# OPTML-Group/Unlearn-Saliency

Measured on AMD Instinct MI355X. Metric: unlearn_steps_per_sec (ResNet-18/CIFAR-10 10%-forget, RL + SalUn mask, batch 256/GPU), higher is better.
Workload: dtype f32

## Files before the change

### include/salun.h

```cpp
#ifndef SALUN_H
#define SALUN_H

#include <stddef.h>
#include <stdint.h>

#ifdef __cplusplus
extern "C" {
#endif

#define SALUN_OK 0
#define SALUN_EINVAL (-22)
#define SALUN_ENOSPC (-28)
#define SALUN_EIO (-5)

#define SALUN_MAX_THRESHOLDS 16

typedef void *salun_stream_t;

int salun_version(void);
const char *salun_strerror(int code);
const char *salun_arch(void);
int salun_clock_probe(unsigned long long *out , int samples, int spins, salun_stream_t stream);

int salun_saliency_accumulate(float *acc , const float *g ,
// ... 163 lines not shown
                       float *lse , int B, int H, int Nq, int Nk, int D, long long q_bs, int q_ld,
                       long long k_bs, int k_ld, long long v_bs, int v_ld, long long o_bs, int o_ld, double scale,
                       salun_stream_t stream);
int salun_attn_backward(const uint16_t *q , const uint16_t *k , const uint16_t *v ,
                        const uint16_t *o , const uint16_t *d_o , const float *lse ,
                        uint16_t *dq , uint16_t *dk , uint16_t *dv , float *dsum , int B, int H,
                        int Nq, int Nk, int D, long long q_bs, int q_ld, long long k_bs, int k_ld, long long v_bs, int v_ld,
                        long long o_bs, int o_ld, long long do_bs, int do_ld, double scale, salun_stream_t stream);

size_t salun_ln_bf16_workspace_bytes(int64_t rows, int C);
int salun_ln_bf16_forward(const uint16_t *x , const float *gamma , const float *beta ,
                          uint16_t *y , float *stats , int64_t rows, int C, double eps,
                          salun_stream_t stream);
int salun_ln_bf16_backward(const uint16_t *dy , const uint16_t *x , const float *gamma ,
                           const float *stats , uint16_t *dx , float *dgamma , float *dbeta ,
                           int64_t rows, int C, int accumulate, void *ws , size_t ws_bytes, salun_stream_t stream);
int salun_geglu_bf16_forward(const uint16_t *h , uint16_t *out , int64_t rows, int F, salun_stream_t stream);
int salun_geglu_bf16_backward(const uint16_t *h , const uint16_t *dy , uint16_t *dh , int64_t rows,
                              int F, salun_stream_t stream);

size_t salun_bn_workspace_bytes(int C);
int salun_bn_forward(const float *x , const float *res , float *y ,
                     const float *gamma , const float *beta , float *running_mean ,
                     float *running_var , long long *num_batches_tracked ,
                     float *save_mean , float *save_invstd ,
                     int N, int C, int HW, int training, double momentum, double eps, int relu, void *ws ,
                     size_t ws_bytes, salun_stream_t stream);
int salun_bn_backward(const float *dy , const float *y , const float *x ,
                      const float *gamma , const float *save_mean , const float *save_invstd ,
                      float *dx , float *dres , float *dgamma , float *dbeta ,
                      float *grad_gamma_acc , float *grad_beta_acc ,
                      int N, int C, int HW, int training, int relu, void *ws , size_t ws_bytes,
                      salun_stream_t stream);

size_t salun_gn_workspace_bytes(int N, int C);
int salun_gn_forward(const float *x , float *y , const float *gamma , const float *beta ,
                     float *save_mean , float *save_rstd , int N, int C, int HW, int G, double eps,
                     int silu, salun_stream_t stream);
int salun_gn_backward(const float *dz , const float *x , const float *gamma ,
                      const float *beta , const float *save_mean , const float *save_rstd ,
                      float *dx , float *dgamma , float *dbeta ,
                      float *grad_gamma_acc , float *grad_beta_acc ,
                      int N, int C, int HW, int G, int silu, void *ws , size_t ws_bytes,
                      salun_stream_t stream);

int salun_gn_backward_fused(const float *dz , const float *x , const float *gamma ,
                            const float *beta , const float *save_mean , const float *save_rstd ,
                            const float *addend , float *dx , float *dgamma ,
                            float *dbeta , float *grad_gamma_acc ,
                            float *grad_beta_acc , float *nk_sum ,
                            float *csum , float *csum_acc , int N, int C, int HW, int G,
                            int silu, void *ws , size_t ws_bytes, salun_stream_t stream);

int salun_param_diff(const float *p , const float *p0 , float *out , int64_t n,
                     salun_stream_t stream);
int salun_soft_threshold_step(float *p , const float *p0 , const float *tau ,
                              int64_t n, salun_stream_t stream);

size_t salun_ewc_workspace_bytes(int64_t n);
int salun_ewc_penalty_grad(const float *p , const float *p_star , const float *F ,
                           float *g , double lambda, float *loss_out , int64_t n,
                           void *ws , size_t ws_bytes, salun_stream_t stream);

int salun_image_batch(const uint8_t *data , const int64_t *idx ,
                      const int32_t *crop , const uint8_t *flip ,
                      float *out , int64_t B, int H, int W, int C, int pad,
// ... 149 lines not shown
```

### unlearn_saliency_amd/_lib.py

```python
from __future__ import annotations

import ctypes
import os
import subprocess

_HERE = os.path.dirname(os.path.abspath(__file__))
LIB_PATH = os.environ.get("SALUN_LIB") or os.path.join(_HERE, "libsalun.so")
CSRC_DIR = os.path.join(_HERE, "csrc")

SALUN_OK = 0
SALUN_EINVAL = -22
SALUN_ENOSPC = -28
SALUN_EIO = -5
SALUN_MAX_THRESHOLDS = 16
SALUN_TOPK_FORCE_FULL_SCAN = 1
SALUN_TOPK_VALUES_ONLY = 2
SALUN_WGRAD_SHARED = 1

c_void_p, c_int, c_int64, c_uint64 = ctypes.c_void_p, ctypes.c_int, ctypes.c_int64, ctypes.c_uint64
c_double, c_size_t = ctypes.c_double, ctypes.c_size_t

class GemmSeg(ctypes.Structure):
    _fields_ = [("A", c_void_p), ("B", c_void_p), ("K", ctypes.c_int32), ("a_i", ctypes.c_int32),
                ("a_k", ctypes.c_int32), ("b_j", ctypes.c_int32), ("b_k", ctypes.c_int32)]
# ... 79 lines not shown
    "salun_conv3x3_pack_weights": (c_int, [c_void_p, c_int, c_void_p]),
    "salun_conv3x3_packed": (c_int, [c_void_p] * 6 + [c_int] * 6 + [c_void_p]),
    "salun_conv2d_backward_weight": (c_int, [c_void_p, c_void_p, c_void_p] + [c_int] * 11 + [c_void_p, c_size_t,
                                                                                          c_void_p]),
    "salun_conv2d_backward_weight_ex": (c_int, [c_void_p, c_void_p, c_void_p] + [c_int] * 11 + [ctypes.c_uint, c_void_p,
                                                                                                 c_size_t, c_void_p]),
    "salun_conv2d_route": (c_int, [c_int] * 11 + [ctypes.c_uint, c_size_t, ctypes.c_char_p, c_size_t,
                                   ctypes.POINTER(c_int)]),
    "salun_conv2d_bf16_supported": (c_int, [c_int] * 5),
    "salun_conv2d_bf16_pack_weights": (c_int, [c_void_p, c_void_p, c_int, c_int, c_int, c_void_p]),
    "salun_bf16_pack_weights_batch": (c_int, [c_void_p, c_int, c_void_p]),
    "salun_conv2d_bf16_data_workspace_bytes": (c_size_t, [c_int] * 8),
    "salun_conv2d_bf16_forward": (c_int, [c_void_p] * 6 + [c_int] * 8 + [c_void_p, c_size_t, c_void_p]),
    "salun_conv2d_bf16_backward_data": (c_int, [c_void_p] * 4 + [c_int] * 8 + [c_void_p, c_size_t, c_void_p]),
    "salun_conv2d_bf16_wgrad_workspace_bytes": (c_size_t, [c_int] * 8),
    "salun_conv2d_bf16_backward_weight": (c_int, [c_void_p] * 4 + [c_int] * 9 + [c_void_p, c_size_t, c_void_p]),
    "salun_colsum_bf16_workspace_bytes": (c_size_t, [c_int]),
    "salun_colsum_bf16": (c_int, [c_void_p, c_void_p, c_void_p, c_int64, c_int, c_int, c_int, c_void_p, c_size_t, c_void_p]),
    "salun_conv2d_bf16_backward_weight_ex": (c_int, [c_void_p] * 5 + [c_int] * 9 + [c_void_p, c_size_t, c_void_p]),
    "salun_gn_bf16_workspace_bytes": (c_size_t, [c_int] * 4),
    "salun_gn_bf16_forward": (c_int, [c_void_p] * 6 + [c_int] * 4 + [c_double, c_int, c_void_p, c_size_t, c_void_p]),
    "salun_gn_bf16_backward": (c_int, [c_void_p] * 8 + [c_int] * 6 + [c_void_p, c_size_t, c_void_p]),
    "salun_attn_supported": (c_int, [c_int]),
    "salun_attn_forward": (c_int, [c_void_p] * 5 + [c_int] * 5 + [ctypes.c_longlong, c_int] * 4 + [c_double, c_void_p]),
    "salun_attn_backward": (c_int, [c_void_p] * 10 + [c_int] * 5 + [ctypes.c_longlong, c_int] * 5 + [c_double, c_void_p]),
    "salun_ln_bf16_workspace_bytes": (c_size_t, [c_int64, c_int]),
    "salun_ln_bf16_forward": (c_int, [c_void_p] * 5 + [c_int64, c_int, c_double, c_void_p]),
    "salun_ln_bf16_backward": (c_int, [c_void_p] * 7 + [c_int64, c_int, c_int, c_void_p, c_size_t, c_void_p]),
    "salun_geglu_bf16_forward": (c_int, [c_void_p, c_void_p, c_int64, c_int, c_void_p]),
    "salun_geglu_bf16_backward": (c_int, [c_void_p, c_void_p, c_void_p, c_int64, c_int, c_void_p]),
    "salun_bn_workspace_bytes": (c_size_t, [c_int]),
    "salun_bn_forward": (c_int, [c_void_p] * 10 + [c_int] * 4 + [c_double, c_double, c_int, c_void_p, c_size_t, c_void_p]),
    "salun_bn_backward": (c_int, [c_void_p] * 12 + [c_int] * 5 + [c_void_p, c_size_t, c_void_p]),
    "salun_conv2d_backward_data_add": (c_int, [c_void_p] * 4 + [c_int] * 10 + [c_void_p]),
    "salun_gn_workspace_bytes": (c_size_t, [c_int, c_int]),
    "salun_gn_forward": (c_int, [c_void_p] * 6 + [c_int] * 4 + [c_double, c_int, c_void_p]),
    "salun_gn_backward": (c_int, [c_void_p] * 11 + [c_int] * 5 + [c_void_p, c_size_t, c_void_p]),
    "salun_gn_backward_fused": (c_int, [c_void_p] * 15 + [c_int] * 5 + [c_void_p, c_size_t, c_void_p]),
    "salun_param_diff": (c_int, [c_void_p, c_void_p, c_void_p, c_int64, c_void_p]),
    "salun_soft_threshold_step": (c_int, [c_void_p, c_void_p, c_void_p, c_int64, c_void_p]),
    "salun_ewc_workspace_bytes": (c_size_t, [c_int64]),
    "salun_ewc_penalty_grad": (c_int, [c_void_p] * 4 + [c_double, c_void_p, c_int64, c_void_p, c_size_t, c_void_p]),
    "salun_image_batch": (c_int, [c_void_p, c_void_p, c_void_p, c_void_p, c_void_p, c_int64, c_int, c_int, c_int,
                                  c_int, c_void_p]),
    "salun_gemm_f32_workspace_bytes": (c_size_t, [ctypes.POINTER(GemmJob), c_int, ctypes.POINTER(GemmSeg), c_int, c_int,
                                                  c_int]),
    "salun_gemm_f32": (c_int, [ctypes.POINTER(GemmJob), c_int, ctypes.POINTER(GemmSeg), c_int, c_int, c_int,
                               ctypes.POINTER(c_int64), c_double, c_void_p, c_size_t, c_void_p]),
    "salun_gemm_f32_route": (c_int, [ctypes.POINTER(GemmJob), c_int, ctypes.POINTER(GemmSeg), c_int, c_int, c_int,
                                     ctypes.POINTER(c_int64), c_void_p, c_size_t, ctypes.POINTER(GemmRoute)]),
    "salun_colsum_f32_workspace_bytes": (c_size_t, [c_int64, c_int]),
    "salun_colsum_f32": (c_int, [c_void_p, c_void_p, c_int64, c_int, c_int64, c_int, c_void_p, c_size_t, c_void_p]),
    "salun_softmax_rows": (c_int, [c_void_p, c_int64, c_int, c_int, c_void_p]),
    "salun_softmax_rows_backward": (c_int, [c_void_p, c_void_p, c_int64, c_int, c_int, c_double, c_void_p]),
    "salun_gemm_bf16_supported": (c_int, [c_int64, c_int, c_int]),
    "salun_gemm_bf16_nt": (c_int, [c_void_p, c_void_p, c_void_p, c_void_p, c_void_p, c_int64, c_int, c_int, c_int, c_void_p]),
    "salun_pack_bf16": (c_int, [c_void_p, c_void_p, c_int, c_int, c_int, c_void_p]),
    "salun_gemm_bf16_tn_supported": (c_int, [c_int64, c_int, c_int]),
    "salun_gemm_bf16_tn_workspace_bytes": (c_size_t, [c_int64, c_int, c_int, c_int]),
    "salun_gemm_bf16_tn": (c_int, [c_void_p, c_void_p, c_void_p, c_int64, c_int, c_int, c_int, c_int, c_void_p, c_size_t, c_void_p]),
    "salun_dropout": (c_int, [c_void_p, c_void_p, c_int64, c_int64, c_int64, c_double, c_uint64, c_void_p, c_void_p]),
    "salun_u64_add": (c_int, [c_void_p, c_uint64, c_void_p]),
    "salun_iu_dot_workspace_bytes": (c_size_t, [c_int, c_int64]),
    "salun_iu_conv_dot": (c_int, [c_void_p, c_void_p, c_int, c_int64, c_void_p, c_void_p, c_size_t, c_void_p]),
    "salun_iu_bn_dot": (c_int, [c_void_p] * 4 + [c_double] + [c_void_p] * 4 + [c_int] * 3 + [c_void_p, c_void_p,
                                                                                           c_size_t, c_void_p]),
# ... 75 lines not shown
```

### unlearn_saliency_amd/csrc/salun_norm.hip

```cpp
#include "salun_common.h"

namespace {

constexpr int BN_MAX_SPLIT = 64;


struct BnWalk {
  int n, i, dn, di, hw4;
  __device__ __forceinline__ BnWalk(int n_lo, int hw4_) : hw4(hw4_) {
    const int t = threadIdx.x;
    n = n_lo + t / hw4_;
    i = t - (t / hw4_) * hw4_;
    dn = 256 / hw4_;
    di = 256 - dn * hw4_;
  }
  __device__ __forceinline__ void next() {
    n += dn;
    i += di;
    if (i >= hw4) { i -= hw4; ++n; }
  }
};

__global__ __launch_bounds__(256) void k_bn_stats_partial(const float *__restrict__ x, int N, int C, int HW, int nsplit,
                                                          double *__restrict__ partial) {
  __shared__ double lds[4];
  const int c = blockIdx.x, s = blockIdx.y;
  const int n_lo = (int)((int64_t)N * s / nsplit), n_hi = (int)((int64_t)N * (s + 1) / nsplit);
  float s1 = 0.f, s2 = 0.f;
  double d1 = 0.0, d2 = 0.0;
  const int hw4 = HW >> 2;
  const int work = (n_hi - n_lo) * hw4;
  int it = 0;
// ... 168 lines not shown
  __syncthreads();
  const float mu = mean[c], is = invstd[c];
  const float gi = gamma[c] * is;
  const float kb = sg[0] * inv_m, kg = sg[1] * inv_m;
  const int n_lo = (int)((int64_t)N * s / nsplit), n_hi = (int)((int64_t)N * (s + 1) / nsplit);
  const int hw4 = HW >> 2;
  const int work = (n_hi - n_lo) * hw4;
  BnWalk wk(n_lo, hw4);
#pragma unroll 2
  for (int e = threadIdx.x; e < work; e += 256, wk.next()) {
    const int n = wk.n, i = wk.i;
    const size_t off = ((size_t)n * C + c) * HW;
    float4 g = reinterpret_cast<const float4 *>(dy + off)[i];
    if (RELU) {
      const float4 yv = reinterpret_cast<const float4 *>(y + off)[i];
      g.x = yv.x > 0.f ? g.x : 0.f; g.y = yv.y > 0.f ? g.y : 0.f;
      g.z = yv.z > 0.f ? g.z : 0.f; g.w = yv.w > 0.f ? g.w : 0.f;
    }
    if (DRES) reinterpret_cast<float4 *>(dres + off)[i] = g;
    float4 o;
    if (TRAIN) {
      const float4 xv = reinterpret_cast<const float4 *>(x + off)[i];
      o.x = gi * (g.x - (kb + ((xv.x - mu) * is) * kg));
      o.y = gi * (g.y - (kb + ((xv.y - mu) * is) * kg));
      o.z = gi * (g.z - (kb + ((xv.z - mu) * is) * kg));
      o.w = gi * (g.w - (kb + ((xv.w - mu) * is) * kg));
    } else {
      o.x = gi * g.x; o.y = gi * g.y; o.z = gi * g.z; o.w = gi * g.w;
    }
    reinterpret_cast<float4 *>(dx + off)[i] = o;
  }
}

inline int bn_nsplit(int N, int C) {
  int ns = (1024 + C - 1) / C;
  if (ns > N) ns = N;
  if (ns > BN_MAX_SPLIT) ns = BN_MAX_SPLIT;
  if (ns < 1) ns = 1;
  return ns;
}

}

SALUN_EXPORT size_t salun_bn_workspace_bytes(int C) {
  return sizeof(double) * 2 * (size_t)(C > 0 ? C : 0) * BN_MAX_SPLIT;
}

SALUN_EXPORT int salun_bn_forward(const float *x, const float *res, float *y, const float *gamma, const float *beta,
                                  float *running_mean, float *running_var, long long *num_batches_tracked,
                                  float *save_mean, float *save_invstd, int N, int C, int HW, int training,
                                  double momentum, double eps, int relu, void *ws, size_t ws_bytes,
                                  salun_stream_t stream) {
  if (!x || !y || !gamma || !beta || !save_mean || !save_invstd || N < 1 || C < 1 || HW < 4 || (HW & 3))
    return SALUN_EINVAL;
  if (!training && (!running_mean || !running_var)) return SALUN_EINVAL;
  if (!salun_aligned16(x) || !salun_aligned16(y) || (res && !salun_aligned16(res))) return SALUN_EINVAL;
  hipStream_t st = salun_hip_stream(stream);
  const int ns = bn_nsplit(N, C);
  double *partial = static_cast<double *>(ws);
  if (training) {
    if (!ws || ws_bytes < salun_bn_workspace_bytes(C)) return SALUN_ENOSPC;
    hipLaunchKernelGGL(k_bn_stats_partial, dim3(C, ns), dim3(256), 0, st, x, N, C, HW, ns, partial);
    SALUN_LAUNCH_CHECK();
  }
#define SALUN_BN_APPLY(RELU_, RES_, TRAIN_)                                                                       \
  hipLaunchKernelGGL((k_bn_apply<RELU_, RES_, TRAIN_>), dim3(C, ns), dim3(256), 0, st, x, res, y, partial,         \
                     save_mean, save_invstd, gamma, beta, running_mean, running_var, num_batches_tracked, N, C,  \
                     HW, ns, (float)eps, (float)momentum)
  const bool r = relu != 0, a = res != nullptr, t = training != 0;
  if (r && a && t) SALUN_BN_APPLY(true, true, true);
  else if (r && a) SALUN_BN_APPLY(true, true, false);
  else if (r && t) SALUN_BN_APPLY(true, false, true);
  else if (r) SALUN_BN_APPLY(true, false, false);
  else if (a && t) SALUN_BN_APPLY(false, true, true);
  else if (a) SALUN_BN_APPLY(false, true, false);
  else if (t) SALUN_BN_APPLY(false, false, true);
  else SALUN_BN_APPLY(false, false, false);
#undef SALUN_BN_APPLY
// ... 8 lines not shown
                                   salun_stream_t stream) {
  if (!dy || !x || !gamma || !save_mean || !save_invstd || !dx || !dgamma || !dbeta || N < 1 || C < 1 || HW < 4 ||
      (HW & 3) || (relu && !y))
    return SALUN_EINVAL;
  if (!ws || ws_bytes < salun_bn_workspace_bytes(C)) return SALUN_ENOSPC;
  if (!salun_aligned16(dy) || !salun_aligned16(x) || !salun_aligned16(dx) || (y && !salun_aligned16(y)) ||
      (dres && !salun_aligned16(dres)))
    return SALUN_EINVAL;
  hipStream_t st = salun_hip_stream(stream);
  const int ns = bn_nsplit(N, C);
  double *partial = static_cast<double *>(ws);
  if (relu) hipLaunchKernelGGL(k_bn_bwd_partial<true>, dim3(C, ns), dim3(256), 0, st, dy, y, x, save_mean, save_invstd, N, C, HW, ns, partial);
  else hipLaunchKernelGGL(k_bn_bwd_partial<false>, dim3(C, ns), dim3(256), 0, st, dy, y, x, save_mean, save_invstd, N, C, HW, ns, partial);
  SALUN_LAUNCH_CHECK();
  const float inv_m = (float)(1.0 / ((double)N * HW));
#define SALUN_BN_BWD(RELU_, TRAIN_, DRES_)                                                                          \
  hipLaunchKernelGGL((k_bn_bwd_apply<RELU_, TRAIN_, DRES_>), dim3(C, ns), dim3(256), 0, st, dy, y, x, save_mean,   \
                     save_invstd, gamma, partial, dgamma, dbeta, grad_gamma_acc, grad_beta_acc, dx, dres, N, C, HW, \
                     ns, inv_m)
  const bool r = relu != 0, t = training != 0, d = dres != nullptr;
  if (r && t && d) SALUN_BN_BWD(true, true, true);
  else if (r && t) SALUN_BN_BWD(true, true, false);
  else if (r && d) SALUN_BN_BWD(true, false, true);
  else if (r) SALUN_BN_BWD(true, false, false);
  else if (t && d) SALUN_BN_BWD(false, true, true);
  else if (t) SALUN_BN_BWD(false, true, false);
  else if (d) SALUN_BN_BWD(false, false, true);
  else SALUN_BN_BWD(false, false, false);
#undef SALUN_BN_BWD
  SALUN_LAUNCH_CHECK();
  return SALUN_OK;
}

namespace {

constexpr int GN_ITEMS = 16;
constexpr int GN_MAX_SEG = 1024;

__device__ __forceinline__ float gn_sigmoid(float y) { return 1.0f / (1.0f + expf(-y)); }

__device__ __forceinline__ float seg_sum(float v, int r) {
  for (int off = 1; off < r; off <<= 1) v += __shfl_xor(v, off, 64);
  return v;
}

template <bool SILU, int ITEMS>
__global__ __launch_bounds__(256) void k_gn_fwd(const float *__restrict__ x, float *__restrict__ y,
                                                const float *__restrict__ gamma, const float *__restrict__ beta,
                                                float *__restrict__ mean, float *__restrict__ rstd, int C, int HW,
                                                int G, float eps) {
  constexpr bool CACHED = ITEMS > 0;
  __shared__ double lds[4];
  __shared__ float st[2];
  const int ng = blockIdx.x, n = ng / G, g = ng - n * G;
  const int cpg = C / G;
  const int L = cpg * HW, nvec = L >> 2;
  const size_t base = ((size_t)n * C + (size_t)g * cpg) * HW;
  const float4 *xv = reinterpret_cast<const float4 *>(x + base);
  float4 v[CACHED ? ITEMS : 1];
  float s1 = 0.f, s2 = 0.f;
  double d1 = 0.0, d2 = 0.0;
  if (CACHED) {
#pragma unroll
    for (int i = 0; i < (CACHED ? ITEMS : 1); ++i) {
      const int e = threadIdx.x + i * 256;
      if (e < nvec) v[i] = xv[e];
// ... 349 lines not shown
```

### unlearn_saliency_amd/norm.py

```python
from __future__ import annotations

import torch

from .fastfn import FastFunction
import torch.nn as nn
import torch.nn.functional as F

from . import gradsink, ops


class _FusedBN(FastFunction):
    @staticmethod
    def forward(ctx, x, weight, bias, residual, running_mean, running_var, training, momentum, eps, relu, nbt=None):
        out = ops.bn_forward(x, residual, weight, bias, running_mean, running_var, training, momentum, eps, relu, nbt)
        if out is None:
            raise RuntimeError("fused BN: unsupported shape (H*W must be a multiple of 4)")
        y, mean, invstd = out
        ctx.save_for_backward(x, y if relu else None, weight, bias, mean, invstd)
        ctx.params = (weight, bias)
        ctx.cfg = (bool(training), bool(relu), residual is not None)
        ctx.mark_non_differentiable(mean, invstd)
        return y

    @staticmethod
    def backward(ctx, dy):
        x, y, weight, bias, mean, invstd = ctx.saved_tensors
        training, relu, has_res = ctx.cfg
        gw, gb = gradsink.sink(ctx.params[0]), gradsink.sink(ctx.params[1])
        if gw is None or gb is None:
            gw = gb = None
        dx, dres, dgamma, dbeta = ops.bn_backward(_grad_on_grid(dy), y, x, weight, mean, invstd, training, relu,
                                                  has_res and ctx.needs_input_grad[3], gw, gb)
        if gw is not None:
            gradsink.arrived(weight)
            gradsink.arrived(bias)
            dgamma = dbeta = None
        return dx, dgamma, dbeta, dres, None, None, None, None, None, None, None


def _on_grid(t: torch.Tensor) -> bool:
    return t.data_ptr() % 16 == 0


def _grad_on_grid(dy: torch.Tensor) -> torch.Tensor:
    dy = dy.contiguous()
    return dy if _on_grid(dy) else dy.clone()


def _eligible(x: torch.Tensor, bn: nn.BatchNorm2d) -> bool:
    return (type(bn) is nn.BatchNorm2d and x.is_cuda and x.dtype == torch.float32 and x.dim() == 4 and (x.shape[2] * x.shape[3]) % 4 == 0
            and bn.affine and bn.track_running_stats and bn.momentum is not None and not torch.is_autocast_enabled())


def fused_bn_act(x: torch.Tensor, bn: nn.BatchNorm2d, residual: torch.Tensor = None, relu: bool = True):
    ok = _eligible(x, bn) and (not x.is_contiguous() or _on_grid(x)) and \
        (residual is None or not residual.is_contiguous() or _on_grid(residual))
    if not ok:
        y = bn(x)
        if residual is not None:
            y = y + residual
        return F.relu(y) if relu else y
    x = x.contiguous()
    if residual is not None:
        residual = residual.contiguous()
    return _FusedBN.apply(x, bn.weight, bn.bias, residual, bn.running_mean, bn.running_var, bn.training,
# ... 91 lines not shown
```

### unlearn_saliency_amd/ops.py

```python
from __future__ import annotations

import ctypes
from typing import Optional, Sequence

import torch

from .fastfn import FastFunction

from . import _lib, ringpack, weightimg
from ._lib import c_double, c_int, c_int64, c_size_t, c_uint64, c_void_p, check
from .streams import _stream, _stream_handle


def _dev(t: Optional[torch.Tensor], dtype: torch.dtype, name: str, allow_none: bool = False) -> c_void_p:
    if t is None:
        if allow_none:
            return c_void_p(None)
        raise ValueError(f"{name} must not be None")
    if not t.is_cuda:
        raise RuntimeError(f"{name}: the SalUn HIP kernels need a device tensor (got {t.device}); no CPU fallback")
    if t.dtype != dtype:
        raise TypeError(f"{name}: expected {dtype}, got {t.dtype}")
    if not t.is_contiguous():
        raise ValueError(f"{name} must be contiguous")
# ... 787 lines not shown
                            _dev(gamma, torch.float32, "weight"), _dev(beta, torch.float32, "bias"),
                            _dev(running_mean, torch.float32, "running_mean", True),
                            _dev(running_var, torch.float32, "running_var", True),
                            _dev(num_batches_tracked, torch.int64, "num_batches_tracked", True),
                            c_void_p(mean.data_ptr()),
                            c_void_p(invstd.data_ptr()), N, C, H * W, int(bool(training)), c_double(momentum),
                            c_double(eps), int(bool(relu)), c_void_p(ws.data_ptr()), c_size_t(ws.numel()), _stream())
    if rc == _lib.SALUN_EINVAL:
        return None
    check(rc, "salun_bn_forward")
    return y, mean, invstd


def bn_backward(dy, y, x, gamma, mean, invstd, training, relu, want_dres, gamma_grad_acc=None, beta_grad_acc=None):
    N, C, H, W = x.shape
    L = _lib.lib()
    dx = torch.empty_like(x)
    dres = torch.empty_like(x) if want_dres else None
    dgamma = torch.empty(C, dtype=torch.float32, device=x.device)
    dbeta = torch.empty(C, dtype=torch.float32, device=x.device)
    ws = workspace(L.salun_bn_workspace_bytes(C), x.device)
    check(L.salun_bn_backward(_dev(dy, torch.float32, "dy"), _dev(y, torch.float32, "y", True),
                              _dev(x, torch.float32, "x"), _dev(gamma, torch.float32, "weight"),
                              _dev(mean, torch.float32, "mean"), _dev(invstd, torch.float32, "invstd"),
                              c_void_p(dx.data_ptr()), _dev(dres, torch.float32, "dres", True),
                              c_void_p(dgamma.data_ptr()), c_void_p(dbeta.data_ptr()),
                              _dev(gamma_grad_acc, torch.float32, "gamma.grad", True),
                              _dev(beta_grad_acc, torch.float32, "beta.grad", True), N, C, H * W,
                              int(bool(training)), int(bool(relu)), c_void_p(ws.data_ptr()), c_size_t(ws.numel()),
                              _stream()), "salun_bn_backward")
    return dx, dres, dgamma, dbeta


def gn_forward(x, gamma, beta, groups, eps, silu):
    N, C, H, W = x.shape
    z = torch.empty_like(x)
    mean = torch.empty(N * groups, dtype=torch.float32, device=x.device)
    rstd = torch.empty(N * groups, dtype=torch.float32, device=x.device)
    rc = _lib.lib().salun_gn_forward(_dev(x, torch.float32, "x"), c_void_p(z.data_ptr()),
                                     _dev(gamma, torch.float32, "weight"), _dev(beta, torch.float32, "bias"),
                                     c_void_p(mean.data_ptr()), c_void_p(rstd.data_ptr()), N, C, H * W, int(groups),
                                     c_double(eps), int(bool(silu)), _stream())
    if rc == _lib.SALUN_EINVAL:
        return None
    check(rc, "salun_gn_forward")
    return z, mean, rstd


def gn_backward(dz, x, gamma, beta, mean, rstd, groups, silu, gamma_grad_acc=None, beta_grad_acc=None, addend=None,
                nk_sum: bool = False, csum: bool = False, csum_acc=None):
    N, C, H, W = x.shape
    L = _lib.lib()
    dx = torch.empty_like(x)
    dgamma = torch.empty(C, dtype=torch.float32, device=x.device)
    dbeta = torch.empty(C, dtype=torch.float32, device=x.device)
    ws = workspace(L.salun_gn_workspace_bytes(N, C), x.device)
    if addend is not None and addend.shape != x.shape:
        raise ValueError("gn_backward: addend must have the shape of x")
    want_nk = bool(nk_sum or csum or csum_acc is not None)
    nk = torch.empty((N, C), dtype=torch.float32, device=x.device) if want_nk else None
    cs = torch.empty(C, dtype=torch.float32, device=x.device) if csum else None
    check(L.salun_gn_backward_fused(_dev(dz, torch.float32, "dz"), _dev(x, torch.float32, "x"),
                                    _dev(gamma, torch.float32, "weight"), _dev(beta, torch.float32, "bias"),
                                    _dev(mean, torch.float32, "mean"), _dev(rstd, torch.float32, "rstd"),
                                    _dev(addend, torch.float32, "addend", True),
                                    c_void_p(dx.data_ptr()), c_void_p(dgamma.data_ptr()), c_void_p(dbeta.data_ptr()),
# ... 124 lines not shown
```

### unlearn_saliency_amd/resblock.py

```python
from __future__ import annotations

import torch

from .fastfn import FastFunction
import torch.nn as nn

import os

from . import dist as sdist
from . import draws, gradsink, ops, wgrad_side

FWD_SHORTCUT_BESIDE = os.environ.get("SALUN_FWD_SHORTCUT_BESIDE", "1") != "0"


def _bn_args(bn: nn.BatchNorm2d):
    return bn.running_mean, bn.running_var, bn.training, bn.momentum, bn.eps


class _BasicBlockFn(FastFunction):
    @staticmethod
    def forward(ctx, x, blk, w1, g1, b1, w2, g2, b2, wd, gd, bd):
        s = blk.conv1.stride[0]
        N, C, H, W = x.shape
        P, Q = (H + 2 - 3) // s + 1, (W + 2 - 3) // s + 1
        training = blk.bn1.training
        cd = md = idd = None
        fork = None
        if wd is not None:
            def shortcut():
                cd_ = ops.conv2d_forward(x, wd, None, s, 0, P, Q)
                return (cd_,) + tuple(ops.bn_forward(cd_, None, gd, bd, *_bn_args(blk.downsample[1]), False,
                                                     blk.downsample[1].num_batches_tracked))
            if (FWD_SHORTCUT_BESIDE and wgrad_side.OVERLAP and x.is_cuda
                    and not torch.cuda.is_current_stream_capturing()):
                main, fork = torch.cuda.current_stream(x.device), wgrad_side.stream(x.device)
                fork.wait_stream(main)
                with torch.cuda.stream(fork):
                    cd, skip, md, idd = shortcut()
                x.record_stream(fork)
        c1 = ops.conv2d_forward(x, w1, None, s, 1, P, Q)
        y1, m1, i1 = ops.bn_forward(c1, None, g1, b1, *_bn_args(blk.bn1), True, blk.bn1.num_batches_tracked)
        c2 = ops.conv2d_forward(y1, w2, None, 1, 1, P, Q)
        if wd is None:
            skip = x
        elif fork is None:
            cd, skip, md, idd = shortcut()
        else:
            main.wait_stream(fork)
            for t in (cd, skip, md, idd):
                if t is not None:
                    t.record_stream(main)
        out, m2, i2 = ops.bn_forward(c2, skip, g2, b2, *_bn_args(blk.bn2), True, blk.bn2.num_batches_tracked)
        ctx.save_for_backward(x, c1, y1, c2, out, cd, w1, g1, b1, w2, g2, b2, wd, gd, bd, m1, i1, m2, i2, md, idd)
        ctx.cfg = (s, training)
        return out

    @staticmethod
    def backward(ctx, dout):
        x, c1, y1, c2, out, cd, w1, g1, b1, w2, g2, b2, wd, gd, bd, m1, i1, m2, i2, md, idd = ctx.saved_tensors
        s, training = ctx.cfg
        dout = dout.contiguous()
        grads = {}

        def bn_bwd(dy, y, xin, g, b, m, i, relu, want_dres):
            gw, gb = gradsink.sink(g), gradsink.sink(b)
            if gw is None or gb is None:
                gw = gb = None
            dx, dres, dg, db = ops.bn_backward(dy, y, xin, g, m, i, training, relu, want_dres, gw, gb)
            if gw is not None:
                gradsink.arrived(g)
                gradsink.arrived(b)
                dg = db = None
            return dx, dres, dg, db

        dev = dout.device
        overlap = wgrad_side.OVERLAP

        def wgrad(xin, dy, w, stride, pad):
            dst = gradsink.sink(w)
            if overlap:
                dw = wgrad_side.beside(dev, (xin, dy), lambda side: ops.conv2d_backward_weight(
                    xin, dy, w.shape, stride, pad, out=dst, accumulate=True, shared=True, stream=side), alloc=dst is None)
            else:
                dw = ops.conv2d_backward_weight(xin, dy, w.shape, stride, pad, out=dst, accumulate=True)
            if dst is not None:
                gradsink.arrived(w)
                return None
            return dw

        dc2, dskip, dg2, db2 = bn_bwd(dout, out, c2, g2, b2, m2, i2, True, True)
        dwd = dgd = dbd = None
        dxd = dskip
        if wd is not None:
            dcd, _, dgd, dbd = bn_bwd(dskip, None, cd, gd, bd, md, idd, False, False)
            dwd = wgrad(x, dcd, wd, s, 0)
            dxd = ops.conv2d_backward_data(dcd, wd, x.shape, s, 0) if ctx.needs_input_grad[0] else None
        dw2 = wgrad(y1, dc2, w2, 1, 1)
        dy1 = ops.conv2d_backward_data(dc2, w2, y1.shape, 1, 1)
        dc1, _, dg1, db1 = bn_bwd(dy1, y1, c1, g1, b1, m1, i1, True, False)
        dw1 = wgrad(x, dc1, w1, s, 1)
        dx = ops.conv2d_backward_data(dc1, w1, x.shape, s, 1, addend=dxd) if ctx.needs_input_grad[0] else None
        if overlap and not all(g is None for g in (dw1, dw2, dwd)):
            torch.cuda.current_stream(dev).wait_stream(wgrad_side.stream(dev))
            wgrad_side.release_held(dev)
        return dx, None, dw1, dg1, db1, dw2, dg2, db2, dwd, dgd, dbd


def _probe(blk, shape, device) -> bool:
    N, C, H, W = shape
    s = blk.conv1.stride[0]
    P, Q = (H + 2 - 3) // s + 1, (W + 2 - 3) // s + 1
    K = blk.conv1.out_channels
    if (P * Q) % 4 or (H * W) % 4:
        return False
    e = lambda *sh: torch.empty(sh, dtype=torch.float32, device=device)
    x, y1, dy = e(N, C, H, W), e(N, K, P, Q), e(N, K, P, Q)
    convs = [(x, blk.conv1.weight, s, 1), (y1, blk.conv2.weight, 1, 1)]
    if blk.downsample is not None:
        convs.append((x, blk.downsample[0].weight, s, 0))
    for xin, w, st, pad in convs:
        if ops.conv2d_forward(xin, w, None, st, pad, P, Q) is None:
            return False
        if ops.conv2d_backward_data(dy, w, xin.shape, st, pad, addend=xin) is None:
            return False
        if ops.conv2d_backward_weight(xin, dy, w.shape, st, pad) is None:
            return False
    return True


def _structure_ok(blk) -> bool:
    convs = [blk.conv1, blk.conv2] + ([blk.downsample[0]] if blk.downsample is not None else [])
    bns = [blk.bn1, blk.bn2] + ([blk.downsample[1]] if blk.downsample is not None else [])
# ... 207 lines not shown
```

Before: 117.7.

## Store BN+ReLU activation masks as ballot bitmasks and read them in backward

The fused BN forward kernels now write a per-wave ballot bitmask of positive ReLU outputs, and the backward kernels read these bits instead of the saved f32 output tensor to mask the incoming gradient. This replaces a full-size activation read in the BN backward passes with a much smaller bitmask read. It adds small bitmask writes in forward and more kernel variants. In the residual block the full output tensors are still saved alongside the bits, so memory use grows slightly.

```diff
diff --git a/include/salun.h b/include/salun.h
--- a/include/salun.h
+++ b/include/salun.h
@@ -219,6 +219,20 @@
                       float *grad_gamma_acc , float *grad_beta_acc ,
                       int N, int C, int HW, int training, int relu, void *ws , size_t ws_bytes,
                       salun_stream_t stream);
+size_t salun_bn_relu_bits_bytes(int N, int C, int HW);
+int salun_bn_forward_bits(const float *x , const float *res , float *y ,
+                          const float *gamma , const float *beta , float *running_mean ,
+                          float *running_var , long long *num_batches_tracked ,
+                          float *save_mean , float *save_invstd , void *relu_bits ,
+                          size_t relu_bits_bytes, int N, int C, int HW, int training, double momentum, double eps,
+                          int relu, void *ws , size_t ws_bytes, salun_stream_t stream);
+int salun_bn_backward_bits(const float *dy , const void *relu_bits ,
+                           size_t relu_bits_bytes, const float *x , const float *gamma ,
+                           const float *save_mean , const float *save_invstd , float *dx ,
+                           float *dres , float *dgamma , float *dbeta ,
+                           float *grad_gamma_acc ,
+                           float *grad_beta_acc , int N, int C, int HW, int training,
+                           int relu, void *ws , size_t ws_bytes, salun_stream_t stream);
 
 size_t salun_gn_workspace_bytes(int N, int C);
 int salun_gn_forward(const float *x , float *y , const float *gamma , const float *beta ,
diff --git a/unlearn_saliency_amd/_lib.py b/unlearn_saliency_amd/_lib.py
--- a/unlearn_saliency_amd/_lib.py
+++ b/unlearn_saliency_amd/_lib.py
@@ -135,6 +135,11 @@
     "salun_bn_workspace_bytes": (c_size_t, [c_int]),
     "salun_bn_forward": (c_int, [c_void_p] * 10 + [c_int] * 4 + [c_double, c_double, c_int, c_void_p, c_size_t, c_void_p]),
     "salun_bn_backward": (c_int, [c_void_p] * 12 + [c_int] * 5 + [c_void_p, c_size_t, c_void_p]),
+    "salun_bn_relu_bits_bytes": (c_size_t, [c_int] * 3),
+    "salun_bn_forward_bits": (c_int, [c_void_p] * 11 + [c_size_t] + [c_int] * 4 + [c_double, c_double, c_int, c_void_p,
+                                                                                 c_size_t, c_void_p]),
+    "salun_bn_backward_bits": (c_int, [c_void_p] * 2 + [c_size_t] + [c_void_p] * 10 + [c_int] * 5 + [c_void_p, c_size_t,
+                                                                                                     c_void_p]),
     "salun_conv2d_backward_data_add": (c_int, [c_void_p] * 4 + [c_int] * 10 + [c_void_p]),
     "salun_gn_workspace_bytes": (c_size_t, [c_int, c_int]),
     "salun_gn_forward": (c_int, [c_void_p] * 6 + [c_int] * 4 + [c_double, c_int, c_void_p]),
diff --git a/unlearn_saliency_amd/csrc/salun_norm.hip b/unlearn_saliency_amd/csrc/salun_norm.hip
--- a/unlearn_saliency_amd/csrc/salun_norm.hip
+++ b/unlearn_saliency_amd/csrc/salun_norm.hip
@@ -1,3 +1,5 @@
+#include <type_traits>
+
 #include "salun_common.h"
 
 namespace {
@@ -232,6 +234,248 @@
   }
 }
 
+struct BnWaveWalk {
+  int full, all;
+  size_t word0;
+  __device__ __forceinline__ BnWaveWalk(int work, int c, int s, int nsplit, int max_it) {
+    const int lo = __builtin_amdgcn_readfirstlane((int)(threadIdx.x & ~63u));
+    all = work > lo ? (work - lo + 255) >> 8 : 0;
+    full = work > lo + 63 ? (work - lo - 63 + 255) >> 8 : 0;
+    word0 = (((size_t)c * nsplit + s) * max_it) * 16 + (size_t)(lo >> 6) * 4;
+  }
+};
+
+template <int U>
+struct BnItems : std::integral_constant<int, U> {};
+
+__device__ __forceinline__ float bn_keep(unsigned long long m, float g) {
+  float r;
+  asm("v_cndmask_b32_e64 %0, 0, %1, %2" : "=v"(r) : "v"(g), "s"(m));
+  return r;
+}
+
+__device__ __forceinline__ float4 bn_keep4(const unsigned long long *__restrict__ w, float4 g) {
+  g.x = bn_keep(w[0], g.x); g.y = bn_keep(w[1], g.y); g.z = bn_keep(w[2], g.z); g.w = bn_keep(w[3], g.w);
+  return g;
+}
+
+template <bool RES, bool TRAIN>
+__global__ __launch_bounds__(256) void k_bn_apply_bits(const float *__restrict__ x, const float *__restrict__ res,
+                                                       float *__restrict__ y, const double *__restrict__ partial,
+                                                       float *__restrict__ mean, float *__restrict__ invstd,
+                                                       const float *__restrict__ gamma,
+                                                       const float *__restrict__ beta,
+                                                       float *__restrict__ running_mean,
+                                                       float *__restrict__ running_var,
+                                                       long long *__restrict__ num_batches_tracked, int N, int C,
+                                                       int HW, int nsplit, float eps, float momentum,
+                                                       unsigned long long *__restrict__ bits, int max_it) {
+  __shared__ float st[2];
+  const int c = blockIdx.x, s = blockIdx.y;
+  if (TRAIN) {
+    if (num_batches_tracked && c == 0 && s == 0 && threadIdx.x == 0) *num_batches_tracked += 1;
+    bn_channel_stats(partial, c, nsplit, (double)N * HW, eps, st, s == 0, momentum, mean, invstd, running_mean,
+                     running_var);
+  } else {
+    if (threadIdx.x == 0) {
+      st[0] = running_mean[c];
+      st[1] = 1.0f / sqrtf(running_var[c] + eps);
+      if (s == 0) { mean[c] = st[0]; invstd[c] = st[1]; }
+    }
+    __syncthreads();
+  }
+  const float a = st[1] * gamma[c];
+  const float b = beta[c] - st[0] * a;
+  const int n_lo = (int)((int64_t)N * s / nsplit), n_hi = (int)((int64_t)N * (s + 1) / nsplit);
+  const int hw4 = HW >> 2;
+  const int work = (n_hi - n_lo) * hw4;
+  BnWalk wk(n_lo, hw4);
+  const BnWaveWalk ww(work, c, s, nsplit, max_it);
+  unsigned long long *__restrict__ words = bits + ww.word0;
+  int it = 0;
+  auto step = [&](auto items, const bool partial_it) {
+    constexpr int U = decltype(items)::value;
+    const bool in = !partial_it || (int)threadIdx.x + 256 * it < work;
+    size_t off[U];
+    int pi[U];
+    float4 v[U] = {}, r[U] = {}, o[U];
+    unsigned long long m[U][4];
+#pragma unroll
+    for (int u = 0; u < U; ++u, wk.next()) {
+      off[u] = ((size_t)wk.n * C + c) * HW;
+      pi[u] = wk.i;
+    }
+    if (in) {
+#pragma unroll
+      for (int u = 0; u < U; ++u) {
+        v[u] = reinterpret_cast<const float4 *>(x + off[u])[pi[u]];
+        if (RES) r[u] = reinterpret_cast<const float4 *>(res + off[u])[pi[u]];
+      }
+    }
+#pragma unroll
+    for (int u = 0; u < U; ++u) {
+      o[u].x = v[u].x * a + b; o[u].y = v[u].y * a + b; o[u].z = v[u].z * a + b; o[u].w = v[u].w * a + b;
+      if (RES) { o[u].x += r[u].x; o[u].y += r[u].y; o[u].z += r[u].z; o[u].w += r[u].w; }
+      m[u][0] = __ballot(in && o[u].x > 0.f); m[u][1] = __ballot(in && o[u].y > 0.f);
+      m[u][2] = __ballot(in && o[u].z > 0.f); m[u][3] = __ballot(in && o[u].w > 0.f);
+    }
+    if ((threadIdx.x & 63) == 0) {
+#pragma unroll
+      for (int u = 0; u < U; ++u) {
+        unsigned long long *w = words + (size_t)(it + u) * 16;
+        w[0] = m[u][0]; w[1] = m[u][1]; w[2] = m[u][2]; w[3] = m[u][3];
+      }
+    }
+    if (in) {
+#pragma unroll
+      for (int u = 0; u < U; ++u) {
+        o[u].x = o[u].x > 0.f ? o[u].x : 0.f; o[u].y = o[u].y > 0.f ? o[u].y : 0.f;
+        o[u].z = o[u].z > 0.f ? o[u].z : 0.f; o[u].w = o[u].w > 0.f ? o[u].w : 0.f;
+        reinterpret_cast<float4 *>(y + off[u])[pi[u]] = o[u];
+      }
+    }
+  };
+  for (; it + 2 <= ww.full; it += 2) step(BnItems<2>(), false);
+  for (; it < ww.all; ++it) step(BnItems<1>(), it >= ww.full);
+}
+
+__global__ __launch_bounds__(256) void k_bn_bwd_partial_bits(const float *__restrict__ dy,
+                                                             const unsigned long long *__restrict__ bits, int max_it,
+                                                             const float *__restrict__ x,
+                                                             const float *__restrict__ mean,
+                                                             const float *__restrict__ invstd, int N, int C, int HW,
+                                                             int nsplit, double *__restrict__ partial) {
+  __shared__ double lds[4];
+  const int c = blockIdx.x, s = blockIdx.y;
+  const int n_lo = (int)((int64_t)N * s / nsplit), n_hi = (int)((int64_t)N * (s + 1) / nsplit);
+  const float mu = mean[c], is = invstd[c];
+  float s1 = 0.f, s2 = 0.f;
+  double d1 = 0.0, d2 = 0.0;
+  const int hw4 = HW >> 2;
+  const int work = (n_hi - n_lo) * hw4;
+  BnWalk wk(n_lo, hw4);
+  const BnWaveWalk ww(work, c, s, nsplit, max_it);
+  const unsigned long long *__restrict__ words = bits + ww.word0;
+  int it = 0;
+  auto step = [&](auto items, const bool partial_it) {
+    constexpr int U = decltype(items)::value;
+    const bool in = !partial_it || (int)threadIdx.x + 256 * it < work;
+    float4 g[U] = {}, xv[U] = {};
+    if (in) {
+#pragma unroll
+      for (int u = 0; u < U; ++u, wk.next()) {
+        const size_t off = ((size_t)wk.n * C + c) * HW;
+        g[u] = reinterpret_cast<const float4 *>(dy + off)[wk.i];
+        xv[u] = reinterpret_cast<const float4 *>(x + off)[wk.i];
+      }
+    }
+#pragma unroll
+    for (int u = 0; u < U; ++u) {
+      g[u] = bn_keep4(words + (size_t)(it + u) * 16, g[u]);
+      if (in) {
+        s1 += (g[u].x + g[u].y) + (g[u].z + g[u].w);
+        s2 += (g[u].x * ((xv[u].x - mu) * is) + g[u].y * ((xv[u].y - mu) * is)) +
+              (g[u].z * ((xv[u].z - mu) * is) + g[u].w * ((xv[u].w - mu) * is));
+        if (((it + u) & 7) == 7) { d1 += s1; d2 += s2; s1 = 0.f; s2 = 0.f; }
+      }
+    }
+  };
+  for (; it + 2 <= ww.full; it += 2) step(BnItems<2>(), false);
+  for (; it < ww.all; ++it) step(BnItems<1>(), it >= ww.full);
+  d1 += s1; d2 += s2;
+  const double t1 = salun_block_sum(d1, lds);
+  const double t2 = salun_block_sum(d2, lds);
+  if (threadIdx.x == 0) {
+    partial[((size_t)c * nsplit + s) * 2 + 0] = t1;
+    partial[((size_t)c * nsplit + s) * 2 + 1] = t2;
+  }
+}
+
+template <bool TRAIN, bool DRES>
+__global__ __launch_bounds__(256) void k_bn_bwd_apply_bits(const float *__restrict__ dy,
+                                                           const unsigned long long *__restrict__ bits, int max_it,
+                                                           const float *__restrict__ x,
+                                                           const float *__restrict__ mean,
+                                                           const float *__restrict__ invstd,
+                                                           const float *__restrict__ gamma,
+                                                           const double *__restrict__ partial,
+                                                           float *__restrict__ dgamma, float *__restrict__ dbeta,
+                                                           float *__restrict__ gacc, float *__restrict__ bacc,
+                                                           float *__restrict__ dx, float *__restrict__ dres, int N,
+                                                           int C, int HW, int nsplit, float inv_m) {
+  __shared__ float sg[2];
+  const int c = blockIdx.x, s = blockIdx.y;
+  if (threadIdx.x < 64) {
+    double s1 = 0.0, s2 = 0.0;
+    if ((int)threadIdx.x < nsplit) {
+      s1 = partial[((size_t)c * nsplit + threadIdx.x) * 2 + 0];
+      s2 = partial[((size_t)c * nsplit + threadIdx.x) * 2 + 1];
+    }
+    s1 = salun_wave_sum(s1);
+    s2 = salun_wave_sum(s2);
+    if (threadIdx.x == 0) {
+      sg[0] = (float)s1;
+      sg[1] = (float)s2;
+      if (s == 0) {
+        dbeta[c] = (float)s1;
+        dgamma[c] = (float)s2;
+        if (gacc) gacc[c] += (float)s2;
+        if (bacc) bacc[c] += (float)s1;
+      }
+    }
+  }
+  __syncthreads();
+  const float mu = mean[c], is = invstd[c];
+  const float gi = gamma[c] * is;
+  const float kb = sg[0] * inv_m, kg = sg[1] * inv_m;
+  const int n_lo = (int)((int64_t)N * s / nsplit), n_hi = (int)((int64_t)N * (s + 1) / nsplit);
+  const int hw4 = HW >> 2;
+  const int work = (n_hi - n_lo) * hw4;
+  BnWalk wk(n_lo, hw4);
+  const BnWaveWalk ww(work, c, s, nsplit, max_it);
+  const unsigned long long *__restrict__ words = bits + ww.word0;
+  int it = 0;
+  auto step = [&](auto items, const bool partial_it) {
+    constexpr int U = decltype(items)::value;
+    const bool in = !partial_it || (int)threadIdx.x + 256 * it < work;
+    size_t off[U];
+    int pi[U];
+    float4 g[U] = {}, xv[U] = {};
+#pragma unroll
+    for (int u = 0; u < U; ++u, wk.next()) {
+      off[u] = ((size_t)wk.n * C + c) * HW;
+      pi[u] = wk.i;
+    }
+    if (in) {
+#pragma unroll
+      for (int u = 0; u < U; ++u) {
+        g[u] = reinterpret_cast<const float4 *>(dy + off[u])[pi[u]];
+        if (TRAIN) xv[u] = reinterpret_cast<const float4 *>(x + off[u])[pi[u]];
+      }
+    }
+#pragma unroll
+    for (int u = 0; u < U; ++u) g[u] = bn_keep4(words + (size_t)(it + u) * 16, g[u]);
+    if (in) {
+#pragma unroll
+      for (int u = 0; u < U; ++u) {
+        if (DRES) reinterpret_cast<float4 *>(dres + off[u])[pi[u]] = g[u];
+        float4 o;
+        if (TRAIN) {
+          o.x = gi * (g[u].x - (kb + ((xv[u].x - mu) * is) * kg));
+          o.y = gi * (g[u].y - (kb + ((xv[u].y - mu) * is) * kg));
+          o.z = gi * (g[u].z - (kb + ((xv[u].z - mu) * is) * kg));
+          o.w = gi * (g[u].w - (kb + ((xv[u].w - mu) * is) * kg));
+        } else {
+          o.x = gi * g[u].x; o.y = gi * g[u].y; o.z = gi * g[u].z; o.w = gi * g[u].w;
+        }
+        reinterpret_cast<float4 *>(dx + off[u])[pi[u]] = o;
+      }
+    }
+  };
+  for (; it + 2 <= ww.full; it += 2) step(BnItems<2>(), false);
+  for (; it < ww.all; ++it) step(BnItems<1>(), it >= ww.full);
+}
+
 inline int bn_nsplit(int N, int C) {
   int ns = (1024 + C - 1) / C;
   if (ns > N) ns = N;
@@ -240,10 +484,20 @@
   return ns;
 }
 
+inline int bn_bits_max_it(int N, int C, int HW) {
+  const int ns = bn_nsplit(N, C);
+  return (int)(((int64_t)((N + ns - 1) / ns) * (HW >> 2) + 255) / 256);
+}
+
 }
 
 SALUN_EXPORT size_t salun_bn_workspace_bytes(int C) {
   return sizeof(double) * 2 * (size_t)(C > 0 ? C : 0) * BN_MAX_SPLIT;
+}
+
+SALUN_EXPORT size_t salun_bn_relu_bits_bytes(int N, int C, int HW) {
+  if (N < 1 || C < 1 || HW < 4 || (HW & 3)) return 0;
+  return sizeof(unsigned long long) * 16 * (size_t)C * bn_nsplit(N, C) * bn_bits_max_it(N, C, HW);
 }
 
 SALUN_EXPORT int salun_bn_forward(const float *x, const float *res, float *y, const float *gamma, const float *beta,
@@ -318,6 +572,82 @@
   return SALUN_OK;
 }
 
+SALUN_EXPORT int salun_bn_forward_bits(const float *x, const float *res, float *y, const float *gamma,
+                                       const float *beta, float *running_mean, float *running_var,
+                                       long long *num_batches_tracked, float *save_mean, float *save_invstd,
+                                       void *relu_bits, size_t relu_bits_bytes, int N, int C, int HW, int training,
+                                       double momentum, double eps, int relu, void *ws, size_t ws_bytes,
+                                       salun_stream_t stream) {
+  if (!relu)
+    return salun_bn_forward(x, res, y, gamma, beta, running_mean, running_var, num_batches_tracked, save_mean,
+                            save_invstd, N, C, HW, training, momentum, eps, relu, ws, ws_bytes, stream);
+  if (!x || !y || !gamma || !beta || !save_mean || !save_invstd || N < 1 || C < 1 || HW < 4 || (HW & 3))
+    return SALUN_EINVAL;
+  if (!training && (!running_mean || !running_var)) return SALUN_EINVAL;
+  if (!salun_aligned16(x) || !salun_aligned16(y) || (res && !salun_aligned16(res))) return SALUN_EINVAL;
+  if (!relu_bits || !salun_aligned16(relu_bits)) return SALUN_EINVAL;
+  if (relu_bits_bytes < salun_bn_relu_bits_bytes(N, C, HW)) return SALUN_ENOSPC;
+  if (training && (!ws || ws_bytes < salun_bn_workspace_bytes(C))) return SALUN_ENOSPC;
+  hipStream_t st = salun_hip_stream(stream);
+  const int ns = bn_nsplit(N, C);
+  double *partial = static_cast<double *>(ws);
+  if (training) {
+    hipLaunchKernelGGL(k_bn_stats_partial, dim3(C, ns), dim3(256), 0, st, x, N, C, HW, ns, partial);
+    SALUN_LAUNCH_CHECK();
+  }
+#define SALUN_BN_APPLY(RES_, TRAIN_)                                                                              \
+  hipLaunchKernelGGL((k_bn_apply_bits<RES_, TRAIN_>), dim3(C, ns), dim3(256), 0, st, x, res, y, partial,          \
+                     save_mean, save_invstd, gamma, beta, running_mean, running_var, num_batches_tracked, N, C,  \
+                     HW, ns, (float)eps, (float)momentum, static_cast<unsigned long long *>(relu_bits),           \
+                     bn_bits_max_it(N, C, HW))
+  const bool a = res != nullptr, t = training != 0;
+  if (a && t) SALUN_BN_APPLY(true, true);
+  else if (a) SALUN_BN_APPLY(true, false);
+  else if (t) SALUN_BN_APPLY(false, true);
+  else SALUN_BN_APPLY(false, false);
+#undef SALUN_BN_APPLY
+  SALUN_LAUNCH_CHECK();
+  return SALUN_OK;
+}
+
+SALUN_EXPORT int salun_bn_backward_bits(const float *dy, const void *relu_bits, size_t relu_bits_bytes, const float *x,
+                                        const float *gamma, const float *save_mean, const float *save_invstd,
+                                        float *dx, float *dres, float *dgamma, float *dbeta, float *grad_gamma_acc,
+                                        float *grad_beta_acc, int N, int C, int HW, int training, int relu, void *ws,
+                                        size_t ws_bytes, salun_stream_t stream) {
+  if (!relu)
+    return salun_bn_backward(dy, nullptr, x, gamma, save_mean, save_invstd, dx, dres, dgamma, dbeta, grad_gamma_acc,
+                             grad_beta_acc, N, C, HW, training, relu, ws, ws_bytes, stream);
+  if (!dy || !x || !gamma || !save_mean || !save_invstd || !dx || !dgamma || !dbeta || N < 1 || C < 1 || HW < 4 ||
+      (HW & 3) || !relu_bits)
+    return SALUN_EINVAL;
+  if (!ws || ws_bytes < salun_bn_workspace_bytes(C)) return SALUN_ENOSPC;
+  if (!salun_aligned16(dy) || !salun_aligned16(x) || !salun_aligned16(dx) || !salun_aligned16(relu_bits) ||
+      (dres && !salun_aligned16(dres)))
+    return SALUN_EINVAL;
+  if (relu_bits_bytes < salun_bn_relu_bits_bytes(N, C, HW)) return SALUN_ENOSPC;
+  hipStream_t st = salun_hip_stream(stream);
+  const int ns = bn_nsplit(N, C), max_it = bn_bits_max_it(N, C, HW);
+  double *partial = static_cast<double *>(ws);
+  const unsigned long long *bits = static_cast<const unsigned long long *>(relu_bits);
+  hipLaunchKernelGGL(k_bn_bwd_partial_bits, dim3(C, ns), dim3(256), 0, st, dy, bits, max_it, x, save_mean, save_invstd,
+                     N, C, HW, ns, partial);
+  SALUN_LAUNCH_CHECK();
+  const float inv_m = (float)(1.0 / ((double)N * HW));
+#define SALUN_BN_BWD(TRAIN_, DRES_)                                                                                 \
+  hipLaunchKernelGGL((k_bn_bwd_apply_bits<TRAIN_, DRES_>), dim3(C, ns), dim3(256), 0, st, dy, bits, max_it, x,       \
+                     save_mean, save_invstd, gamma, partial, dgamma, dbeta, grad_gamma_acc, grad_beta_acc, dx, dres, \
+                     N, C, HW, ns, inv_m)
+  const bool t = training != 0, d = dres != nullptr;
+  if (t && d) SALUN_BN_BWD(true, true);
+  else if (t) SALUN_BN_BWD(true, false);
+  else if (d) SALUN_BN_BWD(false, true);
+  else SALUN_BN_BWD(false, false);
+#undef SALUN_BN_BWD
+  SALUN_LAUNCH_CHECK();
+  return SALUN_OK;
+}
+
 namespace {
 
 constexpr int GN_ITEMS = 16;
diff --git a/unlearn_saliency_amd/norm.py b/unlearn_saliency_amd/norm.py
--- a/unlearn_saliency_amd/norm.py
+++ b/unlearn_saliency_amd/norm.py
@@ -12,11 +12,12 @@
 class _FusedBN(FastFunction):
     @staticmethod
     def forward(ctx, x, weight, bias, residual, running_mean, running_var, training, momentum, eps, relu, nbt=None):
-        out = ops.bn_forward(x, residual, weight, bias, running_mean, running_var, training, momentum, eps, relu, nbt)
+        out = ops.bn_forward_bits(x, residual, weight, bias, running_mean, running_var, training, momentum, eps, relu,
+                                  nbt)
         if out is None:
             raise RuntimeError("fused BN: unsupported shape (H*W must be a multiple of 4)")
-        y, mean, invstd = out
-        ctx.save_for_backward(x, y if relu else None, weight, bias, mean, invstd)
+        y, mean, invstd, bits = out
+        ctx.save_for_backward(x, bits, weight, bias, mean, invstd)
         ctx.params = (weight, bias)
         ctx.cfg = (bool(training), bool(relu), residual is not None)
         ctx.mark_non_differentiable(mean, invstd)
@@ -24,13 +25,13 @@
 
     @staticmethod
     def backward(ctx, dy):
-        x, y, weight, bias, mean, invstd = ctx.saved_tensors
+        x, bits, weight, bias, mean, invstd = ctx.saved_tensors
         training, relu, has_res = ctx.cfg
         gw, gb = gradsink.sink(ctx.params[0]), gradsink.sink(ctx.params[1])
         if gw is None or gb is None:
             gw = gb = None
-        dx, dres, dgamma, dbeta = ops.bn_backward(_grad_on_grid(dy), y, x, weight, mean, invstd, training, relu,
-                                                  has_res and ctx.needs_input_grad[3], gw, gb)
+        dx, dres, dgamma, dbeta = ops.bn_backward_bits(_grad_on_grid(dy), bits, x, weight, mean, invstd, training, relu,
+                                                       has_res and ctx.needs_input_grad[3], gw, gb)
         if gw is not None:
             gradsink.arrived(weight)
             gradsink.arrived(bias)
diff --git a/unlearn_saliency_amd/ops.py b/unlearn_saliency_amd/ops.py
--- a/unlearn_saliency_amd/ops.py
+++ b/unlearn_saliency_amd/ops.py
@@ -843,6 +843,58 @@
     return dx, dres, dgamma, dbeta
 
 
+def bn_forward_bits(x, res, gamma, beta, running_mean, running_var, training, momentum, eps, relu,
+                    num_batches_tracked=None):
+    N, C, H, W = x.shape
+    L = _lib.lib()
+    bits = None
+    if relu:
+        nbytes = L.salun_bn_relu_bits_bytes(N, C, H * W)
+        if nbytes == 0:
+            return None
+        bits = torch.empty(nbytes, dtype=torch.uint8, device=x.device)
+    y = torch.empty_like(x)
+    mean = torch.empty(C, dtype=torch.float32, device=x.device)
+    invstd = torch.empty(C, dtype=torch.float32, device=x.device)
+    ws = workspace(L.salun_bn_workspace_bytes(C), x.device)
+    rc = L.salun_bn_forward_bits(_dev(x, torch.float32, "x"), _dev(res, torch.float32, "res", True),
+                                 c_void_p(y.data_ptr()), _dev(gamma, torch.float32, "weight"),
+                                 _dev(beta, torch.float32, "bias"),
+                                 _dev(running_mean, torch.float32, "running_mean", True),
+                                 _dev(running_var, torch.float32, "running_var", True),
+                                 _dev(num_batches_tracked, torch.int64, "num_batches_tracked", True),
+                                 c_void_p(mean.data_ptr()), c_void_p(invstd.data_ptr()),
+                                 _dev(bits, torch.uint8, "bits", True), c_size_t(bits.numel() if relu else 0),
+                                 N, C, H * W, int(bool(training)), c_double(momentum), c_double(eps), int(bool(relu)),
+                                 c_void_p(ws.data_ptr()), c_size_t(ws.numel()), _stream())
+    if rc == _lib.SALUN_EINVAL:
+        return None
+    check(rc, "salun_bn_forward_bits")
+    return y, mean, invstd, bits
+
+
+def bn_backward_bits(dy, bits, x, gamma, mean, invstd, training, relu, want_dres, gamma_grad_acc=None,
+                     beta_grad_acc=None):
+    N, C, H, W = x.shape
+    L = _lib.lib()
+    dx = torch.empty_like(x)
+    dres = torch.empty_like(x) if want_dres else None
+    dgamma = torch.empty(C, dtype=torch.float32, device=x.device)
+    dbeta = torch.empty(C, dtype=torch.float32, device=x.device)
+    ws = workspace(L.salun_bn_workspace_bytes(C), x.device)
+    check(L.salun_bn_backward_bits(_dev(dy, torch.float32, "dy"), _dev(bits, torch.uint8, "bits", True),
+                                   c_size_t(bits.numel() if bits is not None else 0),
+                                   _dev(x, torch.float32, "x"), _dev(gamma, torch.float32, "weight"),
+                                   _dev(mean, torch.float32, "mean"), _dev(invstd, torch.float32, "invstd"),
+                                   c_void_p(dx.data_ptr()), _dev(dres, torch.float32, "dres", True),
+                                   c_void_p(dgamma.data_ptr()), c_void_p(dbeta.data_ptr()),
+                                   _dev(gamma_grad_acc, torch.float32, "gamma.grad", True),
+                                   _dev(beta_grad_acc, torch.float32, "beta.grad", True), N, C, H * W,
+                                   int(bool(training)), int(bool(relu)), c_void_p(ws.data_ptr()), c_size_t(ws.numel()),
+                                   _stream()), "salun_bn_backward_bits")
+    return dx, dres, dgamma, dbeta
+
+
 def gn_forward(x, gamma, beta, groups, eps, silu):
     N, C, H, W = x.shape
     z = torch.empty_like(x)
diff --git a/unlearn_saliency_amd/resblock.py b/unlearn_saliency_amd/resblock.py
--- a/unlearn_saliency_amd/resblock.py
+++ b/unlearn_saliency_amd/resblock.py
@@ -39,7 +39,7 @@
                     cd, skip, md, idd = shortcut()
                 x.record_stream(fork)
         c1 = ops.conv2d_forward(x, w1, None, s, 1, P, Q)
-        y1, m1, i1 = ops.bn_forward(c1, None, g1, b1, *_bn_args(blk.bn1), True, blk.bn1.num_batches_tracked)
+        y1, m1, i1, r1 = ops.bn_forward_bits(c1, None, g1, b1, *_bn_args(blk.bn1), True, blk.bn1.num_batches_tracked)
         c2 = ops.conv2d_forward(y1, w2, None, 1, 1, P, Q)
         if wd is None:
             skip = x
@@ -50,23 +50,24 @@
             for t in (cd, skip, md, idd):
                 if t is not None:
                     t.record_stream(main)
-        out, m2, i2 = ops.bn_forward(c2, skip, g2, b2, *_bn_args(blk.bn2), True, blk.bn2.num_batches_tracked)
-        ctx.save_for_backward(x, c1, y1, c2, out, cd, w1, g1, b1, w2, g2, b2, wd, gd, bd, m1, i1, m2, i2, md, idd)
+        out, m2, i2, r2 = ops.bn_forward_bits(c2, skip, g2, b2, *_bn_args(blk.bn2), True, blk.bn2.num_batches_tracked)
+        ctx.save_for_backward(x, c1, y1, c2, out, cd, w1, g1, b1, w2, g2, b2, wd, gd, bd, m1, i1, m2, i2, md, idd,
+                              r1, r2)
         ctx.cfg = (s, training)
         return out
 
     @staticmethod
     def backward(ctx, dout):
-        x, c1, y1, c2, out, cd, w1, g1, b1, w2, g2, b2, wd, gd, bd, m1, i1, m2, i2, md, idd = ctx.saved_tensors
+        x, c1, y1, c2, out, cd, w1, g1, b1, w2, g2, b2, wd, gd, bd, m1, i1, m2, i2, md, idd, r1, r2 = ctx.saved_tensors
         s, training = ctx.cfg
         dout = dout.contiguous()
         grads = {}
 
-        def bn_bwd(dy, y, xin, g, b, m, i, relu, want_dres):
+        def bn_bwd(dy, bits, xin, g, b, m, i, relu, want_dres):
             gw, gb = gradsink.sink(g), gradsink.sink(b)
             if gw is None or gb is None:
                 gw = gb = None
-            dx, dres, dg, db = ops.bn_backward(dy, y, xin, g, m, i, training, relu, want_dres, gw, gb)
+            dx, dres, dg, db = ops.bn_backward_bits(dy, bits, xin, g, m, i, training, relu, want_dres, gw, gb)
             if gw is not None:
                 gradsink.arrived(g)
                 gradsink.arrived(b)
@@ -88,7 +89,7 @@
                 return None
             return dw
 
-        dc2, dskip, dg2, db2 = bn_bwd(dout, out, c2, g2, b2, m2, i2, True, True)
+        dc2, dskip, dg2, db2 = bn_bwd(dout, r2, c2, g2, b2, m2, i2, True, True)
         dwd = dgd = dbd = None
         dxd = dskip
         if wd is not None:
@@ -97,7 +98,7 @@
             dxd = ops.conv2d_backward_data(dcd, wd, x.shape, s, 0) if ctx.needs_input_grad[0] else None
         dw2 = wgrad(y1, dc2, w2, 1, 1)
         dy1 = ops.conv2d_backward_data(dc2, w2, y1.shape, 1, 1)
-        dc1, _, dg1, db1 = bn_bwd(dy1, y1, c1, g1, b1, m1, i1, True, False)
+        dc1, _, dg1, db1 = bn_bwd(dy1, r1, c1, g1, b1, m1, i1, True, False)
         dw1 = wgrad(x, dc1, w1, s, 1)
         dx = ops.conv2d_backward_data(dc1, w1, x.shape, s, 1, addend=dxd) if ctx.needs_input_grad[0] else None
         if overlap and not all(g is None for g in (dw1, dw2, dwd)):
```

New measurement: 119.0 (median of 3 runs). About the same (+1.1%).
